# interactiveaudiolab/emphases

Hardware: AMD Instinct MI355X
Metric: utterances/s (10 s @16 kHz) whole-node (higher is better)
Workload: dtype f32; 1 GPU; 64 synthetic 10 s 16 kHz utterances per GPU, conv config, random word alignments, ragged batch with per-utterance (B=1) semantics (BASELINE.json configs[1]); utterances_per_gpu=64, frames_per_gpu=64000, words_per_gpu=1882, conv_tile=64, launch=hipGraph replay, batches_in_flight=2, parallelism=utterance-sharded x1, exchange=none (one rank)

## Files before the change

emphases_amd/csrc/conv_stack.hip:

```cpp
#include <type_traits>

#include "common.h"

#ifndef STACK_STAMP
#define STACK_STAMP(slot)
#endif

namespace emph {

typedef float f32x4 __attribute__((ext_vector_type(4)));
typedef float f32x2 __attribute__((ext_vector_type(2)));

constexpr int kStackChannels = 80;
constexpr int kStackMTiles = 5;
constexpr int kStackSteps = kStackChannels / 4;
constexpr int kStackChunkSteps = 4;
constexpr int kStackChunks = kStackSteps / kStackChunkSteps;
constexpr int kStackStepFloats = 6 * kStackMTiles * 64;
constexpr int kStackChunkFloats = kStackChunkSteps * kStackStepFloats;
constexpr int kStackWidth = 256;
constexpr int kStackStride = 260;
constexpr int kStackThreads = 768;
constexpr int kStackMaxLayers = 3;
constexpr int kSpanFields = 8;

__host__ __device__ constexpr int stack_lds_floats() {
    return kStackChannels * kStackStride + 2 * kStackChunkFloats +
           kStackMaxLayers * kStackChannels;
}

template <bool WORD_SUMS>
__global__ __launch_bounds__(kStackThreads) void conv1d_stack_kernel(
    const float* __restrict__ x, int64_t ldx, float* __restrict__ y, int64_t ldy,
    const float* __restrict__ packs, const float* __restrict__ biases, int layers,
    int relu_mask, const int32_t* __restrict__ spans, const int32_t* __restrict__ slot_map) {
    extern __shared__ __align__(16) float lds[];
    float* act = lds;
    float* ring = act + kStackChannels * kStackStride;
    float* bias_lds = ring + 2 * kStackChunkFloats;
    const int lane = threadIdx.x & 63;
    const int wave = __builtin_amdgcn_readfirstlane(threadIdx.x >> 6);
    const bool loader = wave >= 8;

    const int4 span_a = reinterpret_cast<const int4*>(spans)[2 * blockIdx.x];
    const int4 span_b = reinterpret_cast<const int4*>(spans)[2 * blockIdx.x + 1];
    const int owned_first = span_a.y;
    const int64_t column = span_a.z;
    const int count = span_a.w;
    const int owned = span_b.x;
    const int c0 = span_b.y;

    constexpr int kPackFloats = kStackSteps * kStackStepFloats;
    const int total_chunks = layers * kStackChunks;
    auto request = [&](int g, int first, int n) {
        const int layer = g / kStackChunks;
        const float* source = packs + static_cast<int64_t>(layer) * kPackFloats +
                              (g - layer * kStackChunks) * kStackChunkFloats;
        float* target = ring + (g & 1) * kStackChunkFloats;
        constexpr int kQuads = kStackChunkFloats / 4;
        const int each = (kQuads / 64 + n - 1) / n;
        for (int k = 0; k < each; ++k) {
            const int from = min(((wave - first) + k * n) * 64, kQuads - 64);
            __builtin_amdgcn_global_load_lds(
                (const __attribute__((address_space(1))) void*)(source + 4 * (from + lane)),
                (__attribute__((address_space(3))) void*)(target + 4 * from), 16, 0, 0);
        }
    };
    STACK_STAMP(0);

    const int last_quad = (count - 1) & ~3;
    auto fetch = [&](int c, int q) {
        const int p = c0 + 4 * q;
#ifdef STACK_NO_ROWS
        return make_float4(float(p), 0.f, 0.f, 0.f);
#endif
        return *reinterpret_cast<const float4*>(
            x + static_cast<int64_t>(c) * ldx + column + min(p, last_quad));
    };
    auto masked = [&](int q, const float4& v) {
        const int p = c0 + 4 * q;
        return make_float4(p < count ? v.x : 0.f, p + 1 < count ? v.y : 0.f,
                           p + 2 < count ? v.z : 0.f, p + 3 < count ? v.w : 0.f);
    };
    auto deposit = [&](int c, int q, const float4& raw) {
        const float4 v = masked(q, raw);
        float* target = act + c * kStackStride + 4 * q;
        target[1] = v.x;
        *reinterpret_cast<f32x2*>(target + 2) = f32x2{v.y, v.z};
        target[4] = v.w;
    };
    constexpr int kEarlyRows = 16;
    if (loader) {
        constexpr int kStage = 16 * 64 / 256;
        static_assert(kStage == 4, "the s_waitcnt below count these loads");
        f32x4 rows[kStackChunks - 1][kStage];
        float side[kStackChunks - 1];
        const int mine = threadIdx.x - 512;
        const int q = mine & 63;
        const int p = c0 + 4 * q;
        const float* source = x + static_cast<int64_t>(mine >> 6) * ldx + column + min(p, last_quad);
        const uint32_t target = static_cast<uint32_t>(reinterpret_cast<uintptr_t>(
            (__attribute__((address_space(3))) float*)(act + (mine >> 6) * kStackStride + 4 * q)));
        const int side_kind = mine < 64 ? (mine & 3) : 3;
        const int side_p = side_kind == 0 ? c0 - 1 : c0 + kStackWidth + side_kind - 1;
        const bool side_real = side_kind < 3 && side_p >= 0 && side_p < count;
        const float* side_source = x + static_cast<int64_t>((mine >> 2) & 15) * ldx + column +
                                   (side_real ? side_p : 0);
        const uint32_t side_target = static_cast<uint32_t>(reinterpret_cast<uintptr_t>(
            (__attribute__((address_space(3))) float*)(
                act + ((mine >> 2) & 15) * kStackStride +
                (side_kind == 0 ? 0 : kStackWidth + side_kind))));
        auto ask = [&](int chunk) {
#pragma unroll
            for (int round = 0; round < kStage; ++round) {
                const float* address = source + static_cast<int64_t>(16 * chunk + 4 * round) * ldx;
                asm volatile("global_load_dwordx4 %0, %1, off"
                             : "=v"(rows[chunk - 1][round]) : "v"(address) : "memory");
            }
            const float* address = side_source + static_cast<int64_t>(16 * chunk) * ldx;
            asm volatile("global_load_dword %0, %1, off" : "=v"(side[chunk - 1]) : "v"(address) : "memory");
        };
        auto hand_over = [&](int chunk) {
#pragma unroll
            for (int round = 0; round < kStage; ++round) {
                const f32x4 raw = rows[chunk - 1][round];
                const float first = p < count ? raw[0] : 0.f;
                const f32x2 middle = {p + 1 < count ? raw[1] : 0.f, p + 2 < count ? raw[2] : 0.f};
                const float last = p + 3 < count ? raw[3] : 0.f;
                const uint32_t address = target + (16 * chunk + 4 * round) * (kStackStride * 4);
                asm volatile(
                    "ds_write_b32 %0, %1 offset:4\n\t"
                    "ds_write_b64 %0, %2 offset:8\n\t"
                    "ds_write_b32 %0, %3 offset:16"
                    :
                    : "v"(address), "v"(first), "v"(middle), "v"(last)
                    : "memory");
            }
            const float beside = side_real ? side[chunk - 1] : 0.f;
            const uint32_t address = side_target + 16 * chunk * (kStackStride * 4);
            asm volatile("ds_write_b32 %0, %1" : : "v"(address), "v"(beside) : "memory");
        };
#define EMPH_ROWS_HERE(COUNT, STAGE)                                                        \
    asm volatile("s_waitcnt vmcnt(" #COUNT ")"                                              \
                 : "+v"(rows[STAGE][0]), "+v"(rows[STAGE][1]), "+v"(rows[STAGE][2]),        \
                   "+v"(rows[STAGE][3]), "+v"(side[STAGE])::"memory")
        request(1, 8, 4);
        ask(1);
        __builtin_amdgcn_s_barrier();
        ask(2);
        EMPH_ROWS_HERE(5, 0);
        hand_over(1);
        asm volatile("s_waitcnt lgkmcnt(0)" ::: "memory");
        __builtin_amdgcn_s_barrier();
        request(2, 8, 4);
        ask(3);
        EMPH_ROWS_HERE(13, 1);
        hand_over(2);
        asm volatile("s_waitcnt vmcnt(5) lgkmcnt(0)" ::: "memory");
        __builtin_amdgcn_s_barrier();
        request(3, 8, 4);
        ask(4);
        EMPH_ROWS_HERE(13, 2);
        hand_over(3);
        asm volatile("s_waitcnt vmcnt(5) lgkmcnt(0)" ::: "memory");
        __builtin_amdgcn_s_barrier();
        request(4, 8, 4);
        EMPH_ROWS_HERE(8, 3);
        hand_over(4);
#undef EMPH_ROWS_HERE
        for (int g = 4; g < total_chunks; ++g) {
            asm volatile("s_waitcnt vmcnt(0) lgkmcnt(0)" ::: "memory");
            STACK_STAMP(2 + 8 * (g / kStackChunks) + g % kStackChunks);
            __syncthreads();
            if (g + 1 < total_chunks) request(g + 1, 8, 4);
            if ((g + 1) % kStackChunks == 0 && g + 1 < total_chunks) __syncthreads();
        }
        return;
    }
    request(0, 0, 8);
    {
        static_assert(kStackMaxLayers * kStackChannels <= 512, "one bias per thread");
        const bool has_bias = threadIdx.x < layers * kStackChannels;
        const float bias_value = has_bias ? biases[threadIdx.x] : 0.f;
        constexpr int kEarly = kEarlyRows * 64 / 512;
        float4 early[kEarly];
#pragma unroll
        for (int round = 0; round < kEarly; ++round) {
            const int index = threadIdx.x + 512 * round;
            early[round] = fetch(index >> 6, index & 63);
        }
        float side = 0.f;
        const int side_row = threadIdx.x >> 2, side_kind = threadIdx.x & 3;
        if (side_row < kEarlyRows) {
            const float* row = x + static_cast<int64_t>(side_row) * ldx + column;
            const int p = side_kind == 0 ? c0 - 1 : c0 + kStackWidth + side_kind - 1;
            if (side_kind < 3 && p >= 0 && p < count) side = row[p];
        }
#pragma unroll
        for (int round = 0; round < kEarly; ++round) {
            const int index = threadIdx.x + 512 * round;
            deposit(index >> 6, index & 63, early[round]);
        }
        if (side_row < kEarlyRows)
            act[side_row * kStackStride + (side_kind == 0 ? 0 : kStackWidth + side_kind)] = side;
        if (has_bias) bias_lds[threadIdx.x] = bias_value;
    }
    STACK_STAMP(1);

    const int kk = lane >> 4;
    const int col = lane & 15;
    const int tile = wave & 3;
    const int part = wave >> 2;
    constexpr int split = (kStackMTiles + 1) >> 1;
    const int m_begin = part ? split : 0;
    const float* lane_rows = act + kk * kStackStride + 64 * tile + 4 * col;
    const int p_quad = c0 + 64 * tile + 4 * col;

    auto run = [&](auto count_tag) {
        constexpr int COUNT = decltype(count_tag)::value;
        for (int layer = 0; layer < layers; ++layer) {
            f32x4 acc[6][COUNT];
#pragma unroll
            for (int j = 0; j < 6; ++j)
#pragma unroll
                for (int m = 0; m < COUNT; ++m) acc[j][m] = f32x4{0.f, 0.f, 0.f, 0.f};
            float a[6][COUNT], d[6], v[6];
            auto load_b = [&](int step) {
                const float* source = lane_rows + 4 * step * kStackStride;
                const f32x4 first = *reinterpret_cast<const f32x4*>(source);
                const f32x2 second = *reinterpret_cast<const f32x2*>(source + 4);
                d[0] = first[0], d[1] = first[1], d[2] = first[2], d[3] = first[3];
                d[4] = second[0], d[5] = second[1];
            };
            for (int chunk = 0; chunk < kStackChunks; ++chunk) {
                __syncthreads();
                STACK_STAMP(2 + 8 * layer + chunk);
                if (chunk == 0 || layer == 0) load_b(chunk * kStackChunkSteps);
                const float* weights =
                    ring + ((layer * kStackChunks + chunk) & 1) * kStackChunkFloats +
                    (m_begin << 6) + lane;
#pragma unroll
                for (int ks = 0; ks < kStackChunkSteps; ++ks) {
                    const int step = chunk * kStackChunkSteps + ks;
#pragma unroll
                    for (int j = 0; j < 6; ++j)
#pragma unroll
                        for (int m = 0; m < COUNT; ++m)
#ifdef STACK_FEWER_A_READS
                            a[j][m] = (j & 1) ? a[j - 1][m]
                                              : weights[(ks * 6 * kStackMTiles + j * kStackMTiles + m) << 6];
#else
                            a[j][m] = weights[(ks * 6 * kStackMTiles + j * kStackMTiles + m) << 6];
#endif
#ifdef STACK_NO_TRANSFORM
                    for (int j = 0; j < 6; ++j) v[j] = d[j];
#else
                    const float p = fmaf(-4.f, d[2], d[4]);
                    const float q = fmaf(-4.f, d[1], d[3]);
                    const float c = d[4] - d[2];
                    const float e = 2.f * (d[3] - d[1]);
                    v[0] = fmaf(4.f, d[0], fmaf(-5.f, d[2], d[4]));
                    v[1] = p + q;
                    v[2] = p - q;
                    v[3] = c + e;
                    v[4] = c - e;
                    v[5] = fmaf(4.f, d[1], fmaf(-5.f, d[3], d[5]));
#endif
                    if (step + 1 < kStackSteps) load_b(step + 1);
#pragma unroll
                    for (int j = 0; j < 6; ++j)
#pragma unroll
                        for (int m = 0; m < COUNT; ++m)
                            acc[j][m] = __builtin_amdgcn_mfma_f32_16x16x4f32(
                                a[j][m], v[j], acc[j][m], 0, 0, 0);
                }
            }
            const bool relu = (relu_mask >> layer) & 1;
            const bool last = layer == layers - 1;
            const float* bias_row = bias_lds + layer * kStackChannels;
            STACK_STAMP(2 + 8 * layer + 5);
            if (!last) {
                __syncthreads();
#pragma unroll
                for (int m = 0; m < COUNT; ++m) {
                    const int channel0 = 16 * (m_begin + m) + 4 * kk;
                    const f32x4 add = *reinterpret_cast<const f32x4*>(bias_row + channel0);
#pragma unroll
                    for (int r = 0; r < 4; ++r) {
                        const float m1 = acc[1][m][r], m2 = acc[2][m][r];
                        const float m3 = acc[3][m][r], m4 = acc[4][m][r];
                        const float s12 = m1 + m2, d12 = m1 - m2, s34 = m3 + m4, d34 = m3 - m4;
                        float o0 = acc[0][m][r] + s12 + s34 + add[r];
                        float o1 = fmaf(2.f, d34, d12) + add[r];
                        float o2 = fmaf(4.f, s34, s12) + add[r];
                        float o3 = fmaf(8.f, d34, d12) + acc[5][m][r] + add[r];
                        if (relu) {
                            o0 = o0 < 0.f ? 0.f : o0;
                            o1 = o1 < 0.f ? 0.f : o1;
                            o2 = o2 < 0.f ? 0.f : o2;
                            o3 = o3 < 0.f ? 0.f : o3;
                        }
                        o0 = p_quad < count ? o0 : 0.f;
                        o1 = p_quad + 1 < count ? o1 : 0.f;
                        o2 = p_quad + 2 < count ? o2 : 0.f;
                        o3 = p_quad + 3 < count ? o3 : 0.f;
                        float* target =
                            act + (channel0 + r) * kStackStride + 64 * tile + 4 * col + 1;
                        target[0] = o0;
                        *reinterpret_cast<f32x2*>(target + 1) = f32x2{o1, o2};
                        target[3] = o3;
                    }
                }
                STACK_STAMP(2 + 8 * layer + 6);
                continue;
            }
            const int t = p_quad;
            const int owned_end = owned_first + owned;
            if (WORD_SUMS) {
                int4 slots = {-1, -1, -1, -1};
                if (t < count) slots = *reinterpret_cast<const int4*>(slot_map + column + t);
#pragma unroll
                for (int m = 0; m < COUNT; ++m) {
                    const int channel0 = 16 * (m_begin + m) + 4 * kk;
                    const f32x4 add = *reinterpret_cast<const f32x4*>(bias_row + channel0);
                    f32x4 sum[4];
#pragma unroll
                    for (int r = 0; r < 4; ++r) {
                        const float m1 = acc[1][m][r], m2 = acc[2][m][r];
                        const float m3 = acc[3][m][r], m4 = acc[4][m][r];
                        const float s12 = m1 + m2, d12 = m1 - m2, s34 = m3 + m4, d34 = m3 - m4;
                        float o0 = acc[0][m][r] + s12 + s34 + add[r];
                        float o1 = fmaf(2.f, d34, d12) + add[r];
                        float o2 = fmaf(4.f, s34, s12) + add[r];
                        float o3 = fmaf(8.f, d34, d12) + acc[5][m][r] + add[r];
                        if (relu) {
                            o0 = o0 < 0.f ? 0.f : o0;
                            o1 = o1 < 0.f ? 0.f : o1;
                            o2 = o2 < 0.f ? 0.f : o2;
                            o3 = o3 < 0.f ? 0.f : o3;
                        }
                        o0 = (t >= owned_first && t < owned_end) ? o0 : 0.f;
                        o1 = (t + 1 >= owned_first && t + 1 < owned_end) ? o1 : 0.f;
                        o2 = (t + 2 >= owned_first && t + 2 < owned_end) ? o2 : 0.f;
                        o3 = (t + 3 >= owned_first && t + 3 < owned_end) ? o3 : 0.f;
                        o1 += o0;
                        o2 += o1;
                        o3 += o2;
                        float scan = o3;
                        scan += __builtin_bit_cast(float, __builtin_amdgcn_update_dpp(
                            0, __builtin_bit_cast(int, scan), 0x111, 0xf, 0xf, true));
                        scan += __builtin_bit_cast(float, __builtin_amdgcn_update_dpp(
                            0, __builtin_bit_cast(int, scan), 0x112, 0xf, 0xf, true));
                        scan += __builtin_bit_cast(float, __builtin_amdgcn_update_dpp(
                            0, __builtin_bit_cast(int, scan), 0x114, 0xf, 0xf, true));
                        scan += __builtin_bit_cast(float, __builtin_amdgcn_update_dpp(
                            0, __builtin_bit_cast(int, scan), 0x118, 0xf, 0xf, true));
                        const float before = scan - o3;
                        sum[0][r] = o0 + before;
                        sum[1][r] = o1 + before;
                        sum[2][r] = o2 + before;
                        sum[3][r] = o3 + before;
                    }
#pragma unroll
                    for (int j = 0; j < 4; ++j) {
                        const int slot = j == 0 ? slots.x : j == 1 ? slots.y : j == 2 ? slots.z : slots.w;
                        if (slot >= 0 && t + j >= owned_first && t + j < owned_end)
                            *reinterpret_cast<f32x4*>(y + static_cast<int64_t>(slot) * ldy +
                                                      channel0) = sum[j];
                    }
                }
                continue;
            }
            const bool vector_ok = (ldy & 3) == 0 && (column & 3) == 0 &&
                                   (reinterpret_cast<uintptr_t>(y) & 15) == 0;
#pragma unroll
            for (int m = 0; m < COUNT; ++m) {
                const int channel0 = 16 * (m_begin + m) + 4 * kk;
                const f32x4 add = *reinterpret_cast<const f32x4*>(bias_row + channel0);
#pragma unroll
                for (int r = 0; r < 4; ++r) {
                    const float m1 = acc[1][m][r], m2 = acc[2][m][r];
                    const float m3 = acc[3][m][r], m4 = acc[4][m][r];
                    const float s12 = m1 + m2, d12 = m1 - m2, s34 = m3 + m4, d34 = m3 - m4;
                    float4 out;
                    out.x = acc[0][m][r] + s12 + s34 + add[r];
                    out.y = fmaf(2.f, d34, d12) + add[r];
                    out.z = fmaf(4.f, s34, s12) + add[r];
                    out.w = fmaf(8.f, d34, d12) + acc[5][m][r] + add[r];
                    if (relu) {
                        out.x = out.x < 0.f ? 0.f : out.x;
                        out.y = out.y < 0.f ? 0.f : out.y;
                        out.z = out.z < 0.f ? 0.f : out.z;
                        out.w = out.w < 0.f ? 0.f : out.w;
                    }
                    float* target = y + static_cast<int64_t>(channel0 + r) * ldy + column + t;
                    if (vector_ok && t >= owned_first && t + 3 < owned_end) {
                        *reinterpret_cast<float4*>(target) = out;
                    } else {
                        if (t >= owned_first && t < owned_end) target[0] = out.x;
                        if (t + 1 >= owned_first && t + 1 < owned_end) target[1] = out.y;
                        if (t + 2 >= owned_first && t + 2 < owned_end) target[2] = out.z;
                        if (t + 3 >= owned_first && t + 3 < owned_end) target[3] = out.w;
                    }
                }
            }
            STACK_STAMP(2 + 8 * layer + 6);
        }
    };
    if (part == 0) run(std::integral_constant<int, split>{});
    else run(std::integral_constant<int, kStackMTiles - split>{});
}

}

using namespace emph;

extern "C" {

int32_t emph_conv_stack_max_layers(void) { return kStackMaxLayers; }

int32_t emph_conv_stack_spans(const int64_t* host_counts, const int64_t* host_offsets,
                              int32_t n_segments, int32_t* host_spans) {
    int32_t total = 0;
    for (int32_t segment = 0; segment < n_segments; ++segment) {
        const int64_t count = host_counts[segment];
        if (count <= 0) continue;
        const int64_t quads = (count + 3) / 4;
        int64_t pieces = 1;
        if (quads > 64) {
            pieces = 2;
            while (2 * 63 + (pieces - 2) * 62 < quads) ++pieces;
        }
        const int64_t base = quads / pieces;
        int64_t spare = quads - base * pieces;
        int64_t extra[3] = {0, 0, 0};
        if (pieces > 1) {
            if (spare > 0 && base + 1 <= 63) extra[0] = 1, --spare;
            if (spare > 0 && base + 1 <= 63) extra[1] = 1, --spare;
            extra[2] = spare;
        }
        int64_t done = 0;
        for (int64_t k = 0; k < pieces; ++k) {
            int64_t share = base;
            if (pieces == 1) share = quads;
            else if (k == 0) share += extra[0];
            else if (k == pieces - 1) share += extra[1];
            else if (k <= extra[2]) share += 1;
            if (k == pieces - 1) share = quads - done;
            if (host_spans != nullptr) {
                int32_t* row = host_spans + static_cast<int64_t>(total) * kSpanFields;
                const int64_t first = 4 * done;
                int64_t owned = 4 * share;
                if (first + owned > count) owned = count - first;
                row[0] = segment;
                row[1] = static_cast<int32_t>(first);
                row[2] = static_cast<int32_t>(host_offsets[segment]);
                row[3] = static_cast<int32_t>(count);
                row[4] = static_cast<int32_t>(owned);
                row[5] = static_cast<int32_t>(first > 0 ? first - 4 : 0);
                row[6] = row[7] = 0;
            }
            done += share;
            ++total;
        }
    }
    return total;
}

int emph_conv1d_stack(const float* x, int64_t ldx, float* y, int64_t ldy, const float* packs,
                      const float* biases, int32_t layers, int32_t relu_mask,
                      const int32_t* spans, int32_t n_spans, const int32_t* slot_map,
                      void* stream) {
    if (n_spans == 0) return EMPH_OK;
    EMPH_REQUIRE(x && y && packs && biases && spans, EMPH_EINVAL,
                 "emph_conv1d_stack: null pointer");
    EMPH_REQUIRE(layers >= 1 && layers <= kStackMaxLayers, EMPH_ERANGE,
                 "emph_conv1d_stack: %d layers (1 .. %d)", layers, kStackMaxLayers);
    EMPH_REQUIRE((reinterpret_cast<uintptr_t>(x) & 15) == 0 && (ldx & 3) == 0, EMPH_EINVAL,
                 "emph_conv1d_stack: the input must be 16-byte aligned with ldx a multiple of 4");
    EMPH_REQUIRE(slot_map == nullptr ||
                     ((reinterpret_cast<uintptr_t>(y) & 15) == 0 && (ldy & 3) == 0 &&
                      ldy >= kStackChannels && (reinterpret_cast<uintptr_t>(slot_map) & 15) == 0),
                 EMPH_EINVAL, "emph_conv1d_stack: bad sums buffer or slot map");
    const size_t lds = static_cast<size_t>(stack_lds_floats()) * sizeof(float);
    hipStream_t s = static_cast<hipStream_t>(stream);
    if (slot_map != nullptr) {
        auto kernel = conv1d_stack_kernel<true>;
        static LdsReservation reserved;
        if (int status = reserve_lds(reserved, reinterpret_cast<const void*>(kernel), lds,
                                     "emph_conv1d_stack"))
            return status;
        EMPH_LAUNCH(kernel, dim3(n_spans), dim3(kStackThreads), lds, s, x, ldx, y, ldy, packs,
                    biases, layers, relu_mask, spans, slot_map);
    } else {
        auto kernel = conv1d_stack_kernel<false>;
        static LdsReservation reserved;
        if (int status = reserve_lds(reserved, reinterpret_cast<const void*>(kernel), lds,
                                     "emph_conv1d_stack"))
            return status;
        EMPH_LAUNCH(kernel, dim3(n_spans), dim3(kStackThreads), lds, s, x, ldx, y, ldy, packs,
                    biases, layers, relu_mask, spans, slot_map);
    }
    return check_launch("emph_conv1d_stack");
}

}
```

Measured before the change: 435,700 utterances/s.

## Store Winograd-transformed input tiles in LDS instead of raw activation rows

Moves the Winograd input transform out of the MFMA inner loop. The transformed 6-element tiles are now computed once when activations are written to LDS, by the loader waves and the layer epilogue, using DPP lane shifts for neighbour values and a small edge buffer for tile borders. The inner loop then just reads precomputed head/tail vectors. LDS layout grows to 6 floats per quad with XOR swizzling, and the weight chunk size is halved with the wait counts adjusted to match. This adds an extra barrier, DPP traffic and more LDS footprint, which could lower occupancy or add sync cost.

After: 346,300 utterances/s, median of 2. 20.5% lower.

```diff
diff --git a/emphases_amd/csrc/conv_stack.hip b/emphases_amd/csrc/conv_stack.hip
--- a/emphases_amd/csrc/conv_stack.hip
+++ b/emphases_amd/csrc/conv_stack.hip
@@ -14,19 +14,42 @@
 constexpr int kStackChannels = 80;
 constexpr int kStackMTiles = 5;
 constexpr int kStackSteps = kStackChannels / 4;
-constexpr int kStackChunkSteps = 4;
+constexpr int kStackChunkSteps = 2;
 constexpr int kStackChunks = kStackSteps / kStackChunkSteps;
 constexpr int kStackStepFloats = 6 * kStackMTiles * 64;
 constexpr int kStackChunkFloats = kStackChunkSteps * kStackStepFloats;
 constexpr int kStackWidth = 256;
-constexpr int kStackStride = 260;
+constexpr int kStackQuads = kStackWidth / 4;
+constexpr int kStackRow = 6 * kStackQuads;
+constexpr int kStackTail = 4 * kStackQuads;
+constexpr int kStackStages = kStackChannels / 16;
+constexpr int kStackEdge = 10;
 constexpr int kStackThreads = 768;
 constexpr int kStackMaxLayers = 3;
 constexpr int kSpanFields = 8;
 
 __host__ __device__ constexpr int stack_lds_floats() {
-    return kStackChannels * kStackStride + 2 * kStackChunkFloats +
-           kStackMaxLayers * kStackChannels;
+    return kStackChannels * kStackRow + 2 * kStackChunkFloats +
+           kStackMaxLayers * kStackChannels + kStackChannels * kStackEdge + 64;
+}
+
+__device__ __forceinline__ void stack_transform(const float (&d)[6], f32x4& head, f32x2& tail) {
+    const float p = __fmaf_rn(-4.f, d[2], d[4]);
+    const float q = __fmaf_rn(-4.f, d[1], d[3]);
+    const float c = __fsub_rn(d[4], d[2]);
+    const float e = __fmul_rn(2.f, __fsub_rn(d[3], d[1]));
+    head[0] = __fmaf_rn(4.f, d[0], __fmaf_rn(-5.f, d[2], d[4]));
+    head[1] = __fadd_rn(p, q);
+    head[2] = __fsub_rn(p, q);
+    head[3] = __fadd_rn(c, e);
+    tail[0] = __fsub_rn(c, e);
+    tail[1] = __fmaf_rn(4.f, d[1], __fmaf_rn(-5.f, d[3], d[5]));
+}
+
+template <int CONTROL>
+__device__ __forceinline__ float stack_shift(float value) {
+    return __builtin_bit_cast(float, __builtin_amdgcn_update_dpp(
+        0, __builtin_bit_cast(int, value), CONTROL, 0xf, 0xf, true));
 }
 
 template <bool WORD_SUMS>
@@ -36,8 +59,10 @@
     int relu_mask, const int32_t* __restrict__ spans, const int32_t* __restrict__ slot_map) {
     extern __shared__ __align__(16) float lds[];
     float* act = lds;
-    float* ring = act + kStackChannels * kStackStride;
+    float* ring = act + kStackChannels * kStackRow;
     float* bias_lds = ring + 2 * kStackChunkFloats;
+    float* edge = bias_lds + kStackMaxLayers * kStackChannels;
+    float* dump = edge + kStackChannels * kStackEdge;
     const int lane = threadIdx.x & 63;
     const int wave = __builtin_amdgcn_readfirstlane(threadIdx.x >> 6);
     const bool loader = wave >= 8;
@@ -82,63 +107,88 @@
         return make_float4(p < count ? v.x : 0.f, p + 1 < count ? v.y : 0.f,
                            p + 2 < count ? v.z : 0.f, p + 3 < count ? v.w : 0.f);
     };
-    auto deposit = [&](int c, int q, const float4& raw) {
-        const float4 v = masked(q, raw);
-        float* target = act + c * kStackStride + 4 * q;
-        target[1] = v.x;
-        *reinterpret_cast<f32x2*>(target + 2) = f32x2{v.y, v.z};
-        target[4] = v.w;
+    auto deposit = [&](int c, const float4& raw, float beside) {
+        const float4 v = masked(lane, raw);
+        const float below = stack_shift<0x138>(v.w), above = stack_shift<0x130>(v.x);
+        const float d[6] = {lane == 0 ? beside : below, v.x, v.y, v.z, v.w,
+                            lane == 63 ? beside : above};
+        f32x4 head;
+        f32x2 tail;
+        stack_transform(d, head, tail);
+        float* row = act + c * kStackRow;
+        *reinterpret_cast<f32x4*>(row + 4 * lane) = head;
+        *reinterpret_cast<f32x2*>(row + kStackTail + 2 * (lane ^ ((c & 1) << 4))) = tail;
+        if (lane == 0) edge[c * kStackEdge] = beside;
+        if (lane == 63) edge[c * kStackEdge + kStackEdge - 1] = beside;
     };
     constexpr int kEarlyRows = 16;
     if (loader) {
         constexpr int kStage = 16 * 64 / 256;
         static_assert(kStage == 4, "the s_waitcnt below count these loads");
-        f32x4 rows[kStackChunks - 1][kStage];
-        float side[kStackChunks - 1];
+        static_assert(kStackChunkFloats / 4 / 64 == 15, "the s_waitcnt below count 4 requests a chunk");
+        f32x4 rows[kStackStages - 1][kStage];
+        float side[kStackStages - 1];
         const int mine = threadIdx.x - 512;
-        const int q = mine & 63;
-        const int p = c0 + 4 * q;
-        const float* source = x + static_cast<int64_t>(mine >> 6) * ldx + column + min(p, last_quad);
-        const uint32_t target = static_cast<uint32_t>(reinterpret_cast<uintptr_t>(
-            (__attribute__((address_space(3))) float*)(act + (mine >> 6) * kStackStride + 4 * q)));
-        const int side_kind = mine < 64 ? (mine & 3) : 3;
-        const int side_p = side_kind == 0 ? c0 - 1 : c0 + kStackWidth + side_kind - 1;
-        const bool side_real = side_kind < 3 && side_p >= 0 && side_p < count;
-        const float* side_source = x + static_cast<int64_t>((mine >> 2) & 15) * ldx + column +
-                                   (side_real ? side_p : 0);
-        const uint32_t side_target = static_cast<uint32_t>(reinterpret_cast<uintptr_t>(
-            (__attribute__((address_space(3))) float*)(
-                act + ((mine >> 2) & 15) * kStackStride +
-                (side_kind == 0 ? 0 : kStackWidth + side_kind))));
-        auto ask = [&](int chunk) {
+        const int first_row = mine >> 6;
+        const int p = c0 + 4 * lane;
+        const float* source = x + static_cast<int64_t>(first_row) * ldx + column + min(p, last_quad);
+        auto lds_address = [](const float* pointer) {
+            return static_cast<uint32_t>(reinterpret_cast<uintptr_t>(
+                (const __attribute__((address_space(3))) float*)pointer));
+        };
+        const uint32_t head_target = lds_address(act + first_row * kStackRow + 4 * lane);
+        const uint32_t tail_target = lds_address(
+            act + first_row * kStackRow + kStackTail + 2 * (lane ^ ((first_row & 1) << 4)));
+        const int side_p = lane < 32 ? c0 - 1 : c0 + kStackWidth;
+        const bool side_real = side_p >= 0 && side_p < count;
+        const float* side_source = x + static_cast<int64_t>(4 * (lane & 3) + first_row) * ldx +
+                                   column + (side_real ? side_p : 0);
+        const bool at_end = lane == 0 || lane == 63;
+        const uint32_t edge_target =
+            lds_address(edge + first_row * kStackEdge + (lane == 0 ? 0 : kStackEdge - 1));
+        const uint32_t dump_target = lds_address(dump + lane);
+        auto ask = [&](int stage) {
 #pragma unroll
             for (int round = 0; round < kStage; ++round) {
-                const float* address = source + static_cast<int64_t>(16 * chunk + 4 * round) * ldx;
+                const float* address = source + static_cast<int64_t>(16 * stage + 4 * round) * ldx;
                 asm volatile("global_load_dwordx4 %0, %1, off"
-                             : "=v"(rows[chunk - 1][round]) : "v"(address) : "memory");
-            }
-            const float* address = side_source + static_cast<int64_t>(16 * chunk) * ldx;
-            asm volatile("global_load_dword %0, %1, off" : "=v"(side[chunk - 1]) : "v"(address) : "memory");
+                             : "=v"(rows[stage - 1][round]) : "v"(address) : "memory");
+            }
+            const float* address = side_source + static_cast<int64_t>(16 * stage) * ldx;
+            asm volatile("global_load_dword %0, %1, off" : "=v"(side[stage - 1]) : "v"(address) : "memory");
         };
-        auto hand_over = [&](int chunk) {
+        auto hand_over = [&](int stage) {
+            const float beside = side_real ? side[stage - 1] : 0.f;
 #pragma unroll
             for (int round = 0; round < kStage; ++round) {
-                const f32x4 raw = rows[chunk - 1][round];
-                const float first = p < count ? raw[0] : 0.f;
-                const f32x2 middle = {p + 1 < count ? raw[1] : 0.f, p + 2 < count ? raw[2] : 0.f};
-                const float last = p + 3 < count ? raw[3] : 0.f;
-                const uint32_t address = target + (16 * chunk + 4 * round) * (kStackStride * 4);
+                const f32x4 raw = rows[stage - 1][round];
+                const float x0 = p < count ? raw[0] : 0.f;
+                const float x1 = p + 1 < count ? raw[1] : 0.f;
+                const float x2 = p + 2 < count ? raw[2] : 0.f;
+                const float x3 = p + 3 < count ? raw[3] : 0.f;
+                const float left = __builtin_bit_cast(float, __builtin_amdgcn_readlane(
+                    __builtin_bit_cast(int, beside), round));
+                const float right = __builtin_bit_cast(float, __builtin_amdgcn_readlane(
+                    __builtin_bit_cast(int, beside), 60 + round));
+                const float below = stack_shift<0x138>(x3), above = stack_shift<0x130>(x0);
+                const float d[6] = {lane == 0 ? left : below, x0, x1, x2, x3,
+                                    lane == 63 ? right : above};
+                f32x4 head;
+                f32x2 tail;
+                stack_transform(d, head, tail);
+                const int row = 16 * stage + 4 * round;
+                const uint32_t head_at = head_target + row * (kStackRow * 4);
+                const uint32_t tail_at = tail_target + row * (kStackRow * 4);
+                const uint32_t edge_at = at_end ? edge_target + row * (kStackEdge * 4) : dump_target;
+                const float outside = lane == 0 ? d[0] : d[5];
                 asm volatile(
-                    "ds_write_b32 %0, %1 offset:4\n\t"
-                    "ds_write_b64 %0, %2 offset:8\n\t"
-                    "ds_write_b32 %0, %3 offset:16"
+                    "ds_write_b128 %0, %1\n\t"
+                    "ds_write_b64 %2, %3\n\t"
+                    "ds_write_b32 %4, %5"
                     :
-                    : "v"(address), "v"(first), "v"(middle), "v"(last)
+                    : "v"(head_at), "v"(head), "v"(tail_at), "v"(tail), "v"(edge_at), "v"(outside)
                     : "memory");
             }
-            const float beside = side_real ? side[chunk - 1] : 0.f;
-            const uint32_t address = side_target + 16 * chunk * (kStackStride * 4);
-            asm volatile("ds_write_b32 %0, %1" : : "v"(address), "v"(beside) : "memory");
         };
 #define EMPH_ROWS_HERE(COUNT, STAGE)                                                        \
     asm volatile("s_waitcnt vmcnt(" #COUNT ")"                                              \
@@ -154,23 +204,23 @@
         __builtin_amdgcn_s_barrier();
         request(2, 8, 4);
         ask(3);
-        EMPH_ROWS_HERE(13, 1);
+        EMPH_ROWS_HERE(9, 1);
         hand_over(2);
         asm volatile("s_waitcnt vmcnt(5) lgkmcnt(0)" ::: "memory");
         __builtin_amdgcn_s_barrier();
         request(3, 8, 4);
         ask(4);
-        EMPH_ROWS_HERE(13, 2);
+        EMPH_ROWS_HERE(9, 2);
         hand_over(3);
         asm volatile("s_waitcnt vmcnt(5) lgkmcnt(0)" ::: "memory");
         __builtin_amdgcn_s_barrier();
         request(4, 8, 4);
-        EMPH_ROWS_HERE(8, 3);
+        EMPH_ROWS_HERE(4, 3);
         hand_over(4);
 #undef EMPH_ROWS_HERE
         for (int g = 4; g < total_chunks; ++g) {
             asm volatile("s_waitcnt vmcnt(0) lgkmcnt(0)" ::: "memory");
-            STACK_STAMP(2 + 8 * (g / kStackChunks) + g % kStackChunks);
+            if ((g & 1) == 0) STACK_STAMP(2 + 8 * (g / kStackChunks) + (g % kStackChunks >> 1));
             __syncthreads();
             if (g + 1 < total_chunks) request(g + 1, 8, 4);
             if ((g + 1) % kStackChunks == 0 && g + 1 < total_chunks) __syncthreads();
@@ -184,25 +234,19 @@
         const float bias_value = has_bias ? biases[threadIdx.x] : 0.f;
         constexpr int kEarly = kEarlyRows * 64 / 512;
         float4 early[kEarly];
+        float beside[kEarly];
+        const int side_p = lane == 0 ? c0 - 1 : c0 + kStackWidth;
+        const bool side_real = (lane == 0 || lane == 63) && side_p >= 0 && side_p < count;
 #pragma unroll
         for (int round = 0; round < kEarly; ++round) {
-            const int index = threadIdx.x + 512 * round;
-            early[round] = fetch(index >> 6, index & 63);
-        }
-        float side = 0.f;
-        const int side_row = threadIdx.x >> 2, side_kind = threadIdx.x & 3;
-        if (side_row < kEarlyRows) {
-            const float* row = x + static_cast<int64_t>(side_row) * ldx + column;
-            const int p = side_kind == 0 ? c0 - 1 : c0 + kStackWidth + side_kind - 1;
-            if (side_kind < 3 && p >= 0 && p < count) side = row[p];
-        }
-#pragma unroll
-        for (int round = 0; round < kEarly; ++round) {
-            const int index = threadIdx.x + 512 * round;
-            deposit(index >> 6, index & 63, early[round]);
-        }
-        if (side_row < kEarlyRows)
-            act[side_row * kStackStride + (side_kind == 0 ? 0 : kStackWidth + side_kind)] = side;
+            const int row = wave + 8 * round;
+            early[round] = fetch(row, lane);
+            beside[round] = 0.f;
+            if (side_real) beside[round] = x[static_cast<int64_t>(row) * ldx + column + side_p];
+        }
+#pragma unroll
+        for (int round = 0; round < kEarly; ++round)
+            deposit(wave + 8 * round, early[round], beside[round]);
         if (has_bias) bias_lds[threadIdx.x] = bias_value;
     }
     STACK_STAMP(1);
@@ -213,7 +257,9 @@
     const int part = wave >> 2;
     constexpr int split = (kStackMTiles + 1) >> 1;
     const int m_begin = part ? split : 0;
-    const float* lane_rows = act + kk * kStackStride + 64 * tile + 4 * col;
+    const int quad = 16 * tile + col;
+    const float* lane_head = act + kk * kStackRow + 4 * quad;
+    const float* lane_tail = act + kk * kStackRow + kStackTail + 2 * (quad ^ ((kk & 1) << 4));
     const int p_quad = c0 + 64 * tile + 4 * col;
 
     auto run = [&](auto count_tag) {
@@ -224,17 +270,16 @@
             for (int j = 0; j < 6; ++j)
 #pragma unroll
                 for (int m = 0; m < COUNT; ++m) acc[j][m] = f32x4{0.f, 0.f, 0.f, 0.f};
-            float a[6][COUNT], d[6], v[6];
+            float a[6][COUNT], v[6];
+            f32x4 head;
+            f32x2 tail;
             auto load_b = [&](int step) {
-                const float* source = lane_rows + 4 * step * kStackStride;
-                const f32x4 first = *reinterpret_cast<const f32x4*>(source);
-                const f32x2 second = *reinterpret_cast<const f32x2*>(source + 4);
-                d[0] = first[0], d[1] = first[1], d[2] = first[2], d[3] = first[3];
-                d[4] = second[0], d[5] = second[1];
+                head = *reinterpret_cast<const f32x4*>(lane_head + 4 * step * kStackRow);
+                tail = *reinterpret_cast<const f32x2*>(lane_tail + 4 * step * kStackRow);
             };
             for (int chunk = 0; chunk < kStackChunks; ++chunk) {
                 __syncthreads();
-                STACK_STAMP(2 + 8 * layer + chunk);
+                if ((chunk & 1) == 0) STACK_STAMP(2 + 8 * layer + (chunk >> 1));
                 if (chunk == 0 || layer == 0) load_b(chunk * kStackChunkSteps);
                 const float* weights =
                     ring + ((layer * kStackChunks + chunk) & 1) * kStackChunkFloats +
@@ -252,20 +297,8 @@
 #else
                             a[j][m] = weights[(ks * 6 * kStackMTiles + j * kStackMTiles + m) << 6];
 #endif
-#ifdef STACK_NO_TRANSFORM
-                    for (int j = 0; j < 6; ++j) v[j] = d[j];
-#else
-                    const float p = fmaf(-4.f, d[2], d[4]);
-                    const float q = fmaf(-4.f, d[1], d[3]);
-                    const float c = d[4] - d[2];
-                    const float e = 2.f * (d[3] - d[1]);
-                    v[0] = fmaf(4.f, d[0], fmaf(-5.f, d[2], d[4]));
-                    v[1] = p + q;
-                    v[2] = p - q;
-                    v[3] = c + e;
-                    v[4] = c - e;
-                    v[5] = fmaf(4.f, d[1], fmaf(-5.f, d[3], d[5]));
-#endif
+                    v[0] = head[0], v[1] = head[1], v[2] = head[2], v[3] = head[3];
+                    v[4] = tail[0], v[5] = tail[1];
                     if (step + 1 < kStackSteps) load_b(step + 1);
 #pragma unroll
                     for (int j = 0; j < 6; ++j)
@@ -280,7 +313,6 @@
             const float* bias_row = bias_lds + layer * kStackChannels;
             STACK_STAMP(2 + 8 * layer + 5);
             if (!last) {
-                __syncthreads();
 #pragma unroll
                 for (int m = 0; m < COUNT; ++m) {
                     const int channel0 = 16 * (m_begin + m) + 4 * kk;
@@ -304,11 +336,31 @@
                         o1 = p_quad + 1 < count ? o1 : 0.f;
                         o2 = p_quad + 2 < count ? o2 : 0.f;
                         o3 = p_quad + 3 < count ? o3 : 0.f;
-                        float* target =
-                            act + (channel0 + r) * kStackStride + 64 * tile + 4 * col + 1;
-                        target[0] = o0;
-                        *reinterpret_cast<f32x2*>(target + 1) = f32x2{o1, o2};
-                        target[3] = o3;
+                        acc[0][m][r] = o0, acc[1][m][r] = o1, acc[2][m][r] = o2, acc[3][m][r] = o3;
+                        float* slots = edge + (channel0 + r) * kStackEdge + 2 * tile;
+                        if (col == 0) slots[1] = o0;
+                        if (col == 15) slots[2] = o3;
+                    }
+                }
+                __syncthreads();
+#pragma unroll
+                for (int m = 0; m < COUNT; ++m) {
+                    const int channel0 = 16 * (m_begin + m) + 4 * kk;
+#pragma unroll
+                    for (int r = 0; r < 4; ++r) {
+                        const float beside =
+                            edge[(channel0 + r) * kStackEdge + 2 * tile + (col < 8 ? 0 : 3)];
+                        const float below = stack_shift<0x111>(acc[3][m][r]);
+                        const float above = stack_shift<0x101>(acc[0][m][r]);
+                        const float d[6] = {col == 0 ? beside : below, acc[0][m][r], acc[1][m][r],
+                                            acc[2][m][r], acc[3][m][r], col == 15 ? beside : above};
+                        f32x4 head_out;
+                        f32x2 tail_out;
+                        stack_transform(d, head_out, tail_out);
+                        float* row = act + (channel0 + r) * kStackRow;
+                        *reinterpret_cast<f32x4*>(row + 4 * quad) = head_out;
+                        *reinterpret_cast<f32x2*>(row + kStackTail + 2 * (quad ^ ((r & 1) << 4))) =
+                            tail_out;
                     }
                 }
                 STACK_STAMP(2 + 8 * layer + 6);
```
